# sdmiller/cpu_tsdf

Measured on AMD Instinct MI355X. Metric: integrateCloud throughput, Scene A turntable depth frames, 640x480 -> voxel grid, higher is better.
Workload: dtype f32

## Files before the change

### cpu_tsdf_amd/csrc/tsdf_integrate.hip

```cpp
#include <limits.h>
#include <string.h>
#include <math.h>

#include <algorithm>
#include <cmath>
#include <type_traits>

#include "tsdf_common.h"
#include "tsdf_div.h"
#include "tsdf_buffer.h"
#ifdef TSDF_HIP_TEST_HOOKS
#include "tsdf_hip_test.h"
#endif

#ifndef TSDF_COLOR_PK
#define TSDF_COLOR_PK 2
#endif

typedef float f2 __attribute__((ext_vector_type(2)));
typedef float f4 __attribute__((ext_vector_type(4)));

struct IntegrateArgs {
  float m[12];
  float fxf, fyf, cxf, cyf;
  float hb_u, hb_v;
  float hb_max;
  unsigned kcap, kinc;
  int hinge_fixed;
  int neg_in_window;
  unsigned kmax;
  int wmax_is_int;
  float zmin, zmax;
  float zlo;
  float pos, neg;
  float wmax;
  float pos_over_neg;
  int W, H;
  int ny;
  int plane_rows;
  int qpr;
  int z_global0;
  int zl0;
  int log2TX, TX, TY;
  int rpb;
  unsigned bgra_off;
  int expf_fused_r;
  int ref_cull;
  float cull[24];
  int band_fx, band_fy;
  int implied_d;
  int x_abs0, y_abs0;
  int zfast;
  int64_t pitch;
};

static __device__ __forceinline__ int project_exact(const IntegrateArgs &a, const double *__restrict__ cam,
                                                    float gx, float gy, float gz) {
  const Rcp64 rz = rcp64_prepare((double)gz);
  const int u = (int)(div64((double)gx * cam[0], rz) + cam[2]);
  const int v = (int)(div64((double)gy * cam[1], rz) + cam[3]);
  const bool in = (unsigned)u < (unsigned)a.W && (unsigned)v < (unsigned)a.H;
  return in ? v * a.W + u : -1;
}

template <bool ALLIN = false>
static __device__ __forceinline__ int project_fast(const IntegrateArgs &a, float gx, float gy, float gz,
                                                   bool &ambiguous, uint32_t *margin = nullptr) {
  const float y = __builtin_amdgcn_rcpf(gz);
  const float ru = __builtin_fmaf(gx * a.fxf, y, a.cxf);
  const float rv = __builtin_fmaf(gy * a.fyf, y, a.cyf);
  const int u = (int)ru, v = (int)rv;
  if (ALLIN) {
    *margin = min(__float_as_uint(__builtin_amdgcn_fractf(ru)), __float_as_uint(__builtin_amdgcn_fractf(rv)));
    ambiguous = false;
    return (int)__umul24((unsigned)v, (unsigned)a.W) + u;
  }
  const bool cert = __builtin_amdgcn_fractf(ru) > a.hb_u && __builtin_amdgcn_fractf(rv) > a.hb_v;
  ambiguous = !cert;
  const bool in = (unsigned)u < (unsigned)a.W && (unsigned)v < (unsigned)a.H;
  return in ? (int)__umul24((unsigned)v, (unsigned)a.W) + u : -1;
}

template <int ORDER>
static __device__ __forceinline__ void project_quad_allin(const IntegrateArgs &a, const float (&m)[12], const double *__restrict__ cam,
                                                          const f4 cxv, const f4 ytv, const float (&zt)[3], int (&pix)[4],
                                                          float (&gzs)[4]) {
  const f2 cxa = {cxv.x, cxv.y}, cxb = {cxv.z, cxv.w};
  const float yt[3] = {ytv.x, ytv.y, ytv.z};
  f2 ga[3], gb[3];
#pragma unroll
  for (int q = 0; q < 3; ++q) {
    if (ORDER == TSDF_XFORM_PCL_SSE) {
      ga[q] = cxa * m[4 * q] + yt[q];
      gb[q] = cxb * m[4 * q] + yt[q];
    } else {
      ga[q] = ((cxa * m[4 * q] + yt[q]) + zt[q]) + m[4 * q + 3];
      gb[q] = ((cxb * m[4 * q] + yt[q]) + zt[q]) + m[4 * q + 3];
    }
  }
  const f2 ya = {__builtin_amdgcn_rcpf(ga[2].x), __builtin_amdgcn_rcpf(ga[2].y)};
  const f2 yb = {__builtin_amdgcn_rcpf(gb[2].x), __builtin_amdgcn_rcpf(gb[2].y)};
  const f2 cxf2 = {a.cxf, a.cxf}, cyf2 = {a.cyf, a.cyf};
  const f2 rua = __builtin_elementwise_fma(ga[0] * a.fxf, ya, cxf2), rub = __builtin_elementwise_fma(gb[0] * a.fxf, yb, cxf2);
  const f2 rva = __builtin_elementwise_fma(ga[1] * a.fyf, ya, cyf2), rvb = __builtin_elementwise_fma(gb[1] * a.fyf, yb, cyf2);
  const float ru[4] = {rua.x, rua.y, rub.x, rub.y}, rv[4] = {rva.x, rva.y, rvb.x, rvb.y};
  gzs[0] = ga[2].x, gzs[1] = ga[2].y, gzs[2] = gb[2].x, gzs[3] = gb[2].y;
  uint32_t fu[4], fv[4];
#pragma unroll
  for (int j = 0; j < 4; ++j) {
    fu[j] = __float_as_uint(__builtin_amdgcn_fractf(ru[j]));
    fv[j] = __float_as_uint(__builtin_amdgcn_fractf(rv[j]));
    pix[j] = (int)__umul24((unsigned)(int)rv[j], (unsigned)a.W) + (int)ru[j];
  }
  const uint32_t hb = __float_as_uint(a.hb_max);
  const uint32_t least = min(min(min(fu[0], fv[0]), min(min(fu[1], fv[1]), fu[2])), min(min(fv[2], fu[3]), fv[3]));
  if (!(least > hb)) {
    const float gx[4] = {ga[0].x, ga[0].y, gb[0].x, gb[0].y}, gy[4] = {ga[1].x, ga[1].y, gb[1].x, gb[1].y};
#pragma unroll
    for (int j = 0; j < 4; ++j)
      if (!(min(fu[j], fv[j]) > hb)) pix[j] = project_exact(a, cam, gx[j], gy[j], gzs[j]);
  }
}

static __device__ const uint64_t k_exp2f_tab[32] = {
    0x3ff0000000000000ull, 0x3fefd9b0d3158574ull, 0x3fefb5586cf9890full, 0x3fef9301d0125b51ull, 0x3fef72b83c7d517bull,
    0x3fef54873168b9aaull, 0x3fef387a6e756238ull, 0x3fef1e9df51fdee1ull, 0x3fef06fe0a31b715ull, 0x3feef1a7373aa9cbull,
    0x3feedea64c123422ull, 0x3feece086061892dull, 0x3feebfdad5362a27ull, 0x3feeb42b569d4f82ull, 0x3feeab07dd485429ull,
    0x3feea47eb03a5585ull, 0x3feea09e667f3bcdull, 0x3fee9f75e8ec5f74ull, 0x3feea11473eb0187ull, 0x3feea589994cce13ull,
    0x3feeace5422aa0dbull, 0x3feeb737b0cdc5e5ull, 0x3feec49182a3f090ull, 0x3feed503b23e255dull, 0x3feee89f995ad3adull,
    0x3feeff76f2fb5e47ull, 0x3fef199bdd85529cull, 0x3fef3720dcef9069ull, 0x3fef5818dcfba487ull, 0x3fef7c97337b9b5full,
    0x3fefa4afa2a490daull, 0x3fefd0765b6e4540ull};

static __device__ float tsdf_expf_glibc(float x, bool fused_r) {
  const uint32_t ix = __float_as_uint(x), abstop = (ix >> 20) & 0x7ffu;
  if (abstop >= (0x42b00000u >> 20)) {
    if (ix == 0xff800000u) return 0.f;
    if (abstop >= (0x7f800000u >> 20)) return x + x;
    if (x > 0x1.62e42ep6f) return INFINITY;
    if (x < -0x1.9fe368p6f) return 0.f;
    if (x < -0x1.9d1d9ep6f) return 0x1p-149f;
  }
  const double N = 32., InvLn2N = 0x1.71547652b82fep+0 * N, SHIFT = 0x1.8p+52;
  const double C0 = 0x1.c6af84b912394p-5 / N / N / N, C1 = 0x1.ebfce50fac4f3p-3 / N / N, C2 = 0x1.62e42ff0c52d6p-1 / N;
  const double xd = (double)x;
  double z = InvLn2N * xd;
  double kd = z + SHIFT;
  const uint64_t ki = (uint64_t)__double_as_longlong(kd);
  kd -= SHIFT;
  const double r = fused_r ? __builtin_fma(InvLn2N, xd, -kd) : z - kd;
  const uint64_t t = k_exp2f_tab[ki & 31u] + (ki << 47);
  const double s = __longlong_as_double((long long)t);
  z = C0 * r + C1;
  const double r2 = r * r;
  double y = C2 * r + 1.;
  y = z * r2 + y;
  y = y * s;
  return (float)y;
}

static __device__ __forceinline__ bool reference_cull_keeps(const IntegrateArgs &a, float x, float y, float z) {
  bool keep = true;
#pragma unroll
  for (int k = 0; k < 6; ++k) {
    const float *pl = a.cull + 4 * k;
    keep = keep && ((x * pl[0] + y * pl[1]) + (z * pl[2] + 1.0f * pl[3]) <= 0.f);
  }
  return keep;
}

static __device__ __forceinline__ float div32_fast(float a, const Rcp32 &r) {
  const float q0 = a * r.y;
  const float r0 = __builtin_fmaf(r.nb, q0, a);
  const float q1 = __builtin_fmaf(r0, r.y, q0);
  const float r1 = __builtin_fmaf(r.nb, q1, a);
  return __builtin_fmaf(r1, r.y, q1);
}

static __device__ __forceinline__ bool numerator_ok(float v) {
  const float m = fabsf(v);
  return (m >= 0x1p-100f && m <= 0x1p40f) || __float_as_uint(v) == 0u;
}

template <bool COLOR>
static __device__ __forceinline__ void add_observation_ieee(float &d, float &w, uint32_t &rgb, float dn,
                                                            uint32_t bgra, float wmax) {
  const float wn = 1.f;
  const float wsum = w + wn;
  if (COLOR) {
    uint32_t out = 0;
#pragma unroll
    for (int ch = 0; ch < 3; ++ch) {
      const float c_old = (float)((rgb >> (8 * ch)) & 255u);
      const float c_new = (float)((bgra >> (16 - 8 * ch)) & 255u);
      const float num = w * c_old + wn * c_new;
      out |= ((uint32_t)(uint8_t)(num / wsum)) << (8 * ch);
    }
    rgb = out;
  }
  d = (d * w + dn * wn) / wsum;
  w = wsum;
  if (w > wmax) w = wmax;
}

template <bool COLOR, bool DIST = true>
static __device__ __forceinline__ void add_observation_fast(float &d, float &w, uint32_t &rgb, float dn,
                                                            uint32_t bgra, float wmax, const Rcp32 &rs, uint32_t base = 0u,
                                                            const float *hy_tab = nullptr) {
  const float wsum = w + 1.f;
  if (COLOR) {
#if TSDF_COLOR_PK
    const float hy = hy_tab ? *hy_tab : TSDF_COLOR_PK == 2 ? __builtin_fmaf(0.5f, rs.y, -0.5f) : 0.5f * rs.y;
    const float t0 = __builtin_fmaf(__builtin_fmaf(w, (float)(rgb & 255u), (float)((bgra >> 16) & 255u)), rs.y, hy);
    const float t1 = __builtin_fmaf(__builtin_fmaf(w, (float)((rgb >> 8) & 255u), (float)((bgra >> 8) & 255u)), rs.y, hy);
    const float t2 = __builtin_fmaf(__builtin_fmaf(w, (float)((rgb >> 16) & 255u), (float)(bgra & 255u)), rs.y, hy);
    rgb = __builtin_amdgcn_cvt_pk_u8_f32(t0, 0u, __builtin_amdgcn_cvt_pk_u8_f32(t1, 1u, __builtin_amdgcn_cvt_pk_u8_f32(t2, 2u, base)));
#else
    const float hy = hy_tab ? *hy_tab : 0.5f * rs.y;
    const uint32_t q0 = (uint32_t)__builtin_fmaf(__builtin_fmaf(w, (float)(rgb & 255u), (float)((bgra >> 16) & 255u)), rs.y, hy);
    const uint32_t q1 = (uint32_t)__builtin_fmaf(__builtin_fmaf(w, (float)((rgb >> 8) & 255u), (float)((bgra >> 8) & 255u)), rs.y, hy);
    const uint32_t q2 = (uint32_t)__builtin_fmaf(__builtin_fmaf(w, (float)((rgb >> 16) & 255u), (float)(bgra & 255u)), rs.y, hy);
    rgb = q0 | (q1 << 8) | (q2 << 16) | base;
#endif
  }
  if (DIST) d = div32_fast(d * w + dn, rs);
  w = wsum;
  if (w > wmax) w = wmax;
}

#ifndef TSDF_COLOR_F2
#define TSDF_COLOR_F2 0
#endif
static __device__ __forceinline__ void colour_pair_pk(const f2 w, const uint32_t c0a, const uint32_t c0b, const uint32_t csa, const uint32_t csb,
                                                      const f2 y, const f2 hy, const uint32_t base_a, const uint32_t base_b, uint32_t &cva, uint32_t &cvb) {
  f2 t[3];
#pragma unroll
  for (int ch = 0; ch < 3; ++ch) {
    const f2 o = {(float)((c0a >> (8 * ch)) & 255u), (float)((c0b >> (8 * ch)) & 255u)};
    const f2 n = {(float)((csa >> (16 - 8 * ch)) & 255u), (float)((csb >> (16 - 8 * ch)) & 255u)};
    t[ch] = __builtin_elementwise_fma(__builtin_elementwise_fma(w, o, n), y, hy);
  }
  cva = __builtin_amdgcn_cvt_pk_u8_f32(t[0].x, 0u, __builtin_amdgcn_cvt_pk_u8_f32(t[1].x, 1u, __builtin_amdgcn_cvt_pk_u8_f32(t[2].x, 2u, base_a)));
  cvb = __builtin_amdgcn_cvt_pk_u8_f32(t[0].y, 0u, __builtin_amdgcn_cvt_pk_u8_f32(t[1].y, 1u, __builtin_amdgcn_cvt_pk_u8_f32(t[2].y, 2u, base_b)));
}

static __device__ __forceinline__ bool update_is_safe(float d, float w, float dn) {
  const bool w_ok = fabsf(w - 512.f) <= 512.f && __builtin_amdgcn_fractf(w) == 0.f;
  return w_ok && numerator_ok(d * w + dn);
}


struct BlockCoords {
  unsigned bx, by, bz, gdx, gdy;
};
static __device__ __forceinline__ BlockCoords tsdf_block_coords(int zfast) {
  BlockCoords c;
  c.by = blockIdx.y, c.gdy = gridDim.y;
  c.bx = zfast ? blockIdx.z : blockIdx.x;
  c.bz = zfast ? blockIdx.x : blockIdx.z;
  c.gdx = zfast ? gridDim.z : gridDim.x;
  return c;
}

static __device__ __forceinline__ void tsdf_flags_before(const IntegrateArgs &a, const BlockCoords &bc, const uint8_t *band,
                                                         uint8_t *s_bin, unsigned tid) {
  const int row0 = (int)bc.by * a.rpb * a.TY;
  const int rows = min(a.rpb * a.TY, a.ny - row0);
  const int lf = max(0, a.log2TX - 4), fxb = 1 << lf;
  const int yg0 = (a.y_abs0 + row0) >> 2, yg1 = (a.y_abs0 + row0 + max(rows, 1) - 1) >> 2;
  const int xc0 = (a.x_abs0 + (int)bc.bx * a.TX * 4) >> 6;
  const int n_fl = (yg1 - yg0 + 1) << lf;
  const int n_all = ((a.rpb * a.TY + 3) >> 2) << lf;
  for (int i = (int)tid; i < n_all; i += 256) {
    const int yg = yg0 + (i >> lf), xc = xc0 + (i & (fxb - 1));
    s_bin[i] = i < n_fl && yg < a.band_fy && xc < a.band_fx ? band[((int64_t)(a.zl0 + (int)bc.bz) * a.band_fy + yg) * a.band_fx + xc] : (uint8_t)0;
  }
}
static __device__ __forceinline__ uint64_t tsdf_quiet_passes(const IntegrateArgs &a, const uint8_t *s_bin, unsigned tid) {
  const int lane = (int)(tid & 63u), w0 = (int)(tid & ~63u);
  const int fxb = max(1, a.TX >> 4);
  const int rows_w = max(1, 64 >> a.log2TX), ncell = max(1, min(a.TX, 64) >> 4);
  const int ty0 = w0 >> a.log2TX, c0 = (w0 & (a.TX - 1)) >> 4;
  bool q = lane < a.rpb;
  if (q) {
    for (int rr = 0; rr < rows_w; ++rr)
      for (int c = 0; c < ncell; ++c) q &= s_bin[((ty0 + rr + lane * a.TY) >> 2) * fxb + c0 + c] == 0;
  }
  return __builtin_amdgcn_ballot_w64(q);
}

#ifndef TSDF_GUARD_ON_RESULT
#define TSDF_GUARD_ON_RESULT 1
#endif
#ifndef TSDF_EARLY_VOXEL_LOADS
#define TSDF_EARLY_VOXEL_LOADS 2
#endif

#ifndef TSDF_KTAB
#define TSDF_KTAB 0
#endif
#ifndef TSDF_LEAN_K
#define TSDF_LEAN_K 1
#endif
#ifndef TSDF_SWAR_K
#define TSDF_SWAR_K 1
#endif
#ifndef TSDF_LEAN_BAND
#define TSDF_LEAN_BAND 1
#endif
#ifndef TSDF_AMB_UNROLL
#define TSDF_AMB_UNROLL 1
#endif
#ifndef TSDF_PROJ_F2
#define TSDF_PROJ_F2 1
#endif
struct __attribute__((aligned(16))) KEntry {
  float w;
  float y;
  float hy;
  uint32_t k1;
};
static __device__ __forceinline__ KEntry tsdf_ktab_entry(const IntegrateArgs &a, unsigned k) {
  KEntry e;
  e.w = __builtin_fminf((float)k, a.wmax);
  e.y = rcp32_prepare((float)(k + 1u)).y;
  e.hy = TSDF_COLOR_PK == 2 ? __builtin_fmaf(0.5f, e.y, -0.5f) : 0.5f * e.y;
  e.k1 = min(k << 24, a.kcap) + a.kinc;
  return e;
}
#ifndef TSDF_SKIP_FIXED_HINGE
#define TSDF_SKIP_FIXED_HINGE 1
#endif
#ifndef TSDF_EXP_NO_STORE
#define TSDF_EXP_NO_STORE 0
#endif
#ifndef TSDF_EXP_NO_GATHER
#define TSDF_EXP_NO_GATHER 0
#endif
#ifndef TSDF_EXP_NO_VLOAD
#define TSDF_EXP_NO_VLOAD 0
#endif
#if TSDF_EXP_NO_VLOAD && TSDF_EARLY_VOXEL_LOADS
#error "TSDF_EXP_NO_VLOAD declares the voxel words itself: build it with -DTSDF_EARLY_VOXEL_LOADS=0 (tools/ab_bound.sh does)"
#endif
#if !TSDF_GUARD_ON_RESULT && TSDF_EARLY_VOXEL_LOADS
#error "TSDF_GUARD_ON_RESULT=0 tests the numerator d0 * w0 + dn BEFORE unread distance words are rebuilt from the counts, and with TSDF_EARLY_VOXEL_LOADS those words have no initial value: build that A/B with -DTSDF_EARLY_VOXEL_LOADS=0"
#endif
#ifndef TSDF_GATHER_AUX
#define TSDF_GATHER_AUX 0
#endif
#ifndef TSDF_WPE_MAX
#define TSDF_WPE_MAX 8
#endif
#ifndef TSDF_NO_BAND
#define TSDF_NO_BAND 0
#endif
#ifndef TSDF_BAND_PER_WAVE
#define TSDF_BAND_PER_WAVE 1
#endif
#if TSDF_BAND_PER_WAVE
#define TSDF_BAND_DECL                                                                                     \
  __shared__ __attribute__((aligned(16))) uint8_t s_band_sets[4][1024];                                    \
  reinterpret_cast<u4 *>(&s_band_sets[0][0])[tid] = (u4){0u, 0u, 0u, 0u}
#define TSDF_BAND(i) s_band_sets[threadIdx.x >> 6][i]
#define TSDF_BAND_SYNC() ((void)0)
#define TSDF_BAND_FIRST ((int)(tid & 63u))
#define TSDF_BAND_STEP 64
#else
#define TSDF_BAND_DECL                                                          \
  __shared__ __attribute__((aligned(16))) uint8_t s_band[1024 + 64];            \
  reinterpret_cast<uint32_t *>(s_band)[tid] = 0u, s_band[1024 + (tid & 63u)] = 0
#define TSDF_BAND(i) s_band[i]
#define TSDF_BAND_SYNC() __syncthreads()
#define TSDF_BAND_FIRST ((int)tid)
#define TSDF_BAND_STEP 256
#endif
#ifndef TSDF_RECOMPUTE_PX
#define TSDF_RECOMPUTE_PX 1
#endif
#ifndef TSDF_WPE_PACKED
#define TSDF_WPE_PACKED 7
#endif
#ifndef TSDF_WPE_PACKED_COLOR
#define TSDF_WPE_PACKED_COLOR 8
#endif
#define TSDF_WPE_OF(ORDER, COLOR, FASTPROJ, COUNT, PACKED, ALLIN) \
  ((ALLIN) && !(COUNT) && (PACKED) && (COLOR) && (FASTPROJ) ? TSDF_WPE_PACKED_COLOR : (ALLIN) && !(COUNT) && ((PACKED) || !(COLOR)) ? TSDF_WPE_PACKED : TSDF_WPE_GENERAL)
#ifndef TSDF_WPE_GENERAL
#define TSDF_WPE_GENERAL 7
#endif
#ifndef TSDF_PHASE_TIMER
#define TSDF_PHASE_TIMER 0
#endif
#if TSDF_PHASE_TIMER
#define TSDF_NPHASE 16
__device__ unsigned long long g_phase[1024 * TSDF_NPHASE];
static __device__ __forceinline__ uint32_t tsdf_clock_lo() {
  uint64_t t;
  asm volatile("s_memtime %0\n\ts_waitcnt lgkmcnt(0)" : "=s"(t)::"memory");
  return (uint32_t)t;
}
#define TSDF_NACC 9
#define PT_DECL                                                   \
  uint32_t pt_acc[TSDF_NACC];                                     \
  _Pragma("unroll") for (int i_ = 0; i_ < TSDF_NACC; ++i_) asm volatile("v_mov_b32 %0, 0" : "=v"(pt_acc[i_])); \
  const unsigned pt_blk = (blockIdx.x + blockIdx.y * gridDim.x + blockIdx.z * gridDim.x * gridDim.y) & 1023u; \
  uint32_t pt_prev = tsdf_clock_lo();                             \
  const uint32_t pt_t0 = pt_prev
#define PT_MARK(k)                           \
  do {                                       \
    const uint32_t pt_now = tsdf_clock_lo(); \
    pt_acc[k] += pt_now - pt_prev;           \
    pt_prev = pt_now;                        \
  } while (0)
                    \

#define PT_MARK_OUT(k)                                                                                 \
  do {                                                                                                 \
    const uint32_t pt_now = tsdf_clock_lo();                                                           \
    if ((threadIdx.x & 63u) == 0u) atomicAdd(&g_phase[pt_blk * TSDF_NPHASE + (k)], (unsigned long long)(pt_now - pt_prev)); \
    pt_prev = pt_now;                                                                                  \
  } while (0)
#define PT_COUNT(k) pt_acc[k] += 1u
#define PT_DEP4(a_, b_, c_, d_) asm volatile("" ::"v"(a_), "v"(b_), "v"(c_), "v"(d_) : "memory")
#define PT_DEP1(a_) asm volatile("" ::"v"(a_) : "memory")
#define PT_FLUSH()                                                                                       \
  do {                                                                                                   \
    const uint32_t pt_now = tsdf_clock_lo();                                                             \
    if ((threadIdx.x & 63u) == 0u) {                                                                     \
      atomicAdd(&g_phase[pt_blk * TSDF_NPHASE + 15], (unsigned long long)(pt_now - pt_t0));              \
      _Pragma("unroll") for (int i_ = 0; i_ < TSDF_NACC; ++i_)                                           \
          atomicAdd(&g_phase[pt_blk * TSDF_NPHASE + i_], (unsigned long long)pt_acc[i_]);                \
    }                                                                                                    \
  } while (0)
#else
#define PT_DECL
#define PT_MARK(k)
#define PT_MARK_OUT(k)
#define PT_COUNT(k)
#define PT_DEP4(a_, b_, c_, d_)
#define PT_DEP1(a_)
#define PT_FLUSH()
#endif
template <int ORDER, bool COLOR, bool FASTPROJ, bool COUNT, bool PACKED, bool ALLIN = false, bool LIVE = false>
static __global__ void __launch_bounds__(256) __attribute__((amdgpu_waves_per_eu(TSDF_WPE_OF(ORDER, COLOR, FASTPROJ, COUNT, PACKED, ALLIN) < TSDF_WPE_MAX ? TSDF_WPE_OF(ORDER, COLOR, FASTPROJ, COUNT, PACKED, ALLIN) : TSDF_WPE_MAX, TSDF_WPE_MAX)))
k_integrate(const IntegrateArgs a, float *__restrict__ D, float *__restrict__ Wt, uint32_t *__restrict__ RGB,
            uint8_t *__restrict__ K8, const float *__restrict__ depth, const double *__restrict__ cam,
            const float *__restrict__ ctrx, const float *__restrict__ ctry, const float *__restrict__ ctrz,
            unsigned long long *__restrict__ n_obs, const uint8_t *__restrict__ live, uint8_t *__restrict__ band,
            const uint32_t *__restrict__ row_iv) {
  static_assert(!(ALLIN && LIVE), "the ALLIN instance knows no row intervals");
  const BlockCoords bc = tsdf_block_coords(a.zfast);
  PT_DECL;
  bool strad = false;
  if (LIVE) {
    const unsigned flag = live[bc.bx + bc.gdx * (bc.by + bc.gdy * bc.bz)];
    if (flag == 0u) return;
    strad = flag == 2u;
  }
  const unsigned tid = threadIdx.x;
#if TSDF_KTAB
  __shared__ KEntry s_tab[PACKED ? 256 : 1];
#else
  __shared__ f2 s_rcp[256];
#endif
  __shared__ f4 s_yt[256];
  constexpr bool F2 = TSDF_PROJ_F2 && ALLIN && FASTPROJ;
  constexpr bool LEAN_K1 = TSDF_LEAN_K && !TSDF_KTAB && TSDF_COLOR_PK == 2 && PACKED && COLOR;
  __shared__ f4 s_cx[F2 ? 256 : 1];
  __shared__ uint32_t s_iv[LIVE ? 256 : 1];
  TSDF_BAND_DECL;
#if TSDF_KTAB
  if (PACKED) s_tab[tid] = tsdf_ktab_entry(a, tid);
#else
  if (PACKED) {
    const KEntry e = tsdf_ktab_entry(a, tid);
    s_rcp[tid] = (f2){e.y, e.hy};
  }
#endif
  {
    const int yy = (int)bc.by * a.rpb * a.TY + (int)tid;
    {
      const float cy_ = ctry[yy < a.ny ? yy : a.ny - 1], cz_ = ctrz[a.z_global0 + (int)bc.bz];
      f4 t = {0.f, 0.f, 0.f, 0.f};
#pragma unroll
      for (int q = 0; q < 3; ++q)
        t[q] = ORDER == TSDF_XFORM_PCL_SSE ? cy_ * a.m[4 * q + 1] + (cz_ * a.m[4 * q + 2] + a.m[4 * q + 3]) : a.m[4 * q + 1] * cy_;
      s_yt[tid] = t;
    }
    if (F2) {
      const int xq_ = (int)bc.bx * a.TX + (int)(tid & (unsigned)(a.TX - 1));
      if (xq_ < a.qpr) s_cx[tid] = *reinterpret_cast<const f4 *>(ctrx + xq_ * 4);
    }
    if (LIVE && strad) s_iv[tid] = yy < a.ny ? row_iv[(int64_t)bc.bz * a.ny + yy] : 0u;
  }
  __shared__ uint8_t s_bin[PACKED ? 1024 : 1];
  if (PACKED && a.implied_d) tsdf_flags_before(a, bc, band, s_bin, tid);
  __syncthreads();
  const uint64_t quiet = PACKED && a.implied_d ? tsdf_quiet_passes(a, s_bin, tid) : 0ull;
  PT_MARK_OUT(9);
  const int tx = (int)(tid & (unsigned)(a.TX - 1));
  const int ty = (int)(tid >> a.log2TX);
  const int xq = (int)bc.bx * a.TX + tx;
  const int zl = (int)bc.bz;
  const Rcp32 rneg = rcp32_prepare(a.neg);
  unsigned cnt = 0, chg = 0, imp = 0, rdb = 0;
  const int row0 = (int)bc.by * a.rpb * a.TY;
  const int rows = min(a.rpb * a.TY, a.ny - row0);
  const int64_t e0 = ((int64_t)(a.zl0 + zl) * a.plane_rows + row0) * a.pitch;
  const unsigned span = (unsigned)rows * (unsigned)a.pitch;
  const rsrc_t rsD = make_rsrc(D + e0, span * 4u);
  const rsrc_t rsW = make_rsrc(PACKED ? D : Wt + e0, PACKED ? 0u : span * 4u);
  const rsrc_t rsC = make_rsrc(COLOR ? RGB + e0 : (uint32_t *)D, COLOR ? span * 4u : 0u);
  const rsrc_t rsK = make_rsrc(PACKED && !COLOR ? K8 + e0 : (uint8_t *)D, PACKED && !COLOR ? span : 0u);
  const unsigned npix = (unsigned)a.W * (unsigned)a.H;
  const rsrc_t rsF = make_rsrc(depth, COLOR ? a.bgra_off + npix * 4u : npix * 4u);
  const i4_rsrc rsFi = make_rsrc_2d(depth, 4u, 0xffffffffu);
  if (xq < a.qpr) {
    const int x4 = xq * 4;
    const float cz = ctrz[a.z_global0 + zl];
    const float4 cx4 = *reinterpret_cast<const float4 *>(ctrx + x4);
    const float cxs[4] = {cx4.x, cx4.y, cx4.z, cx4.w};
    float px_[4][3], zt[3];
#pragma unroll
    for (int r = 0; r < 3; ++r) {
#pragma unroll
      for (int j = 0; j < 4; ++j) px_[j][r] = cxs[j] * a.m[4 * r];
      zt[r] = ORDER == TSDF_XFORM_PCL_SSE ? cz * a.m[4 * r + 2] + a.m[4 * r + 3] : a.m[4 * r + 2] * cz;
    }
    const unsigned voff = (unsigned)(ty * (int)a.pitch + x4) * 4u;
    const unsigned row_step = (unsigned)a.TY * (unsigned)a.pitch * 4u;
#if TSDF_EARLY_VOXEL_LOADS
    bool pred_obs = true;
#endif
    for (int r = 0; r < a.rpb; ++r) {
      const int y = row0 + ty + r * a.TY;
      if (y >= a.ny) break;
      unsigned iv_lo = 0u, iv_len = 0u;
      if (LIVE && strad) {
        const uint32_t iv = s_iv[ty + r * a.TY];
        iv_lo = iv & 0xffffu, iv_len = iv >> 16;
        if (!((unsigned)(x4 + 3) - iv_lo < iv_len + 3u)) continue;
      }
      const unsigned soff = (unsigned)r * row_step;
      const f4 ytv = s_yt[ty + r * a.TY];
      const float yt[3] = {ytv.x, ytv.y, ytv.z};
#if TSDF_RECOMPUTE_PX
      float px[4][3];
      if constexpr (!F2) {
        float cxr[4] = {cxs[0], cxs[1], cxs[2], cxs[3]};
#pragma unroll
        for (int j = 0; j < 4; ++j) asm volatile("" : "+v"(cxr[j]));
#pragma unroll
        for (int q = 0; q < 3; ++q)
#pragma unroll
          for (int j = 0; j < 4; ++j) px[j][q] = cxr[j] * a.m[4 * q];
      }
#else
      const float (&px)[4][3] = px_;
#endif
      auto transform = [&](int j, int q) -> float {
        if (ORDER == TSDF_XFORM_PCL_SSE) return px[j][q] + yt[q];
        return ((px[j][q] + yt[q]) + zt[q]) + a.m[4 * q + 3];
      };
      int pix[4];
      float gzs[4];
      bool any = false, lowz = false;
      if constexpr (F2) {
        asm volatile("" ::: "memory");
        project_quad_allin<ORDER>(a, a.m, cam, s_cx[tid], ytv, zt, pix, gzs);
        PT_DEP4(pix[0], pix[1], pix[2], pix[3]);
        PT_MARK(0);
      } else {
      unsigned amb_mask = 0;
      uint32_t margin[4] = {0u, 0u, 0u, 0u};
#pragma unroll
      for (int j = 0; j < 4; ++j) {
        const float gx = transform(j, 0), gy = transform(j, 1), gz = transform(j, 2);
        const bool in = ALLIN || (gz > a.zlo && !(gz > a.zmax) && (!LIVE || !strad || (unsigned)(x4 + j) - iv_lo < iv_len));
        gzs[j] = gz;
        if (!ALLIN) lowz |= in && gz < 0x1p-14f;
        int p;
        if (FASTPROJ) {
          bool amb;
          p = project_fast<ALLIN>(a, gx, gy, gz, amb, &margin[j]);
          if (amb && in) amb_mask |= 1u << j;
        } else {
          p = project_exact(a, cam, gx, gy, in ? gz : 1.f);
        }
        pix[j] = in ? p : -1;
        any |= in;
      }
      if (!ALLIN && !any) continue;
      if (ALLIN && FASTPROJ) {
        const uint32_t hb = __float_as_uint(a.hb_max);
        if (!(min(min(margin[0], margin[1]), min(margin[2], margin[3])) > hb)) {
#pragma unroll
          for (int j = 0; j < 4; ++j)
            if (!(margin[j] > hb)) amb_mask |= 1u << j;
        }
      }
#if TSDF_AMB_UNROLL
      if (FASTPROJ && amb_mask) {
#pragma unroll
        for (int j = 0; j < 4; ++j)
          if (amb_mask >> j & 1u) pix[j] = project_exact(a, cam, transform(j, 0), transform(j, 1), transform(j, 2));
      }
#else
      while (FASTPROJ && amb_mask) {
        const int j = __builtin_ctz(amb_mask);
        amb_mask &= amb_mask - 1;
        float g[3];
#pragma unroll
        for (int q = 0; q < 3; ++q)
          g[q] = j == 0 ? transform(0, q) : j == 1 ? transform(1, q) : j == 2 ? transform(2, q) : transform(3, q);
        const int p = project_exact(a, cam, g[0], g[1], g[2]);
        if (j == 0) pix[0] = p;
        if (j == 1) pix[1] = p;
        if (j == 2) pix[2] = p;
        if (j == 3) pix[3] = p;
      }
#endif
      }
#if TSDF_EARLY_VOXEL_LOADS
      constexpr bool EARLY = PACKED;
      const bool d_read = !PACKED || !(r < 64 && (quiet >> r & 1ull));
      u4 d4;
      asm volatile("" : "=v"(d4));
      u4 w4 = {0u, 0u, 0u, 0u}, c4 = {0u, 0u, 0u, 0u};
      uint32_t k4 = 0u;
      const bool ask_early = EARLY && (TSDF_EARLY_VOXEL_LOADS != 2 || pred_obs);
      if (ask_early) {
        if (d_read) d4 = bload128(rsD, voff, soff);
        if (COLOR) c4 = bload128(rsC, voff, soff);
        if (!COLOR) k4 = bload32(rsK, voff >> 2, soff >> 2);
        if (COUNT) rdb += (d_read ? 16u : 0u) + (COLOR ? 16u : 4u);
      }
#endif
      float zs[4];
      uint32_t cs[4] = {0u, 0u, 0u, 0u};
#pragma unroll
      for (int j = 0; j < 4; ++j) {
        if (TSDF_EXP_NO_GATHER) {
          zs[j] = 1e3f + (float)(pix[j] & 1);
          cs[j] = 0x00406080u + (unsigned)pix[j];
        } else if (ALLIN) {
          zs[j] = __uint_as_float(tsdf_struct_buffer_load_u32(rsFi, pix[j], 0, 0, TSDF_GATHER_AUX));
          if (COLOR) cs[j] = tsdf_struct_buffer_load_u32(rsFi, pix[j], 0, (int)a.bgra_off, TSDF_GATHER_AUX);
        } else {
          zs[j] = __uint_as_float(bload32(rsF, (unsigned)pix[j] << 2, 0u));
          if (COLOR) cs[j] = bload32(rsF, (unsigned)pix[j] << 2, a.bgra_off);
        }
      }
// ... 96 lines not shown
          kw[j] = COLOR ? c0[j] : (k4 << (24 - 8 * j));
#if TSDF_KTAB
          const KEntry e = s_tab[kw[j] >> 24];
          w0[j] = e.w, ky[j] = e.y, khy[j] = e.hy, k1[j] = e.k1;
#else
          if (TSDF_LEAN_K && ALLIN) {
            w0[j] = (float)(kw[j] >> 24);
            if (COLOR) asm volatile("" : "+v"(w0[j]));
          } else {
            w0[j] = __builtin_fminf((float)(kw[j] >> 24), a.wmax);
          }
          k1[j] = LEAN_K1 ? min(kw[j], a.kcap | 0xffffffu) + a.kinc : min(kw[j] & 0xff000000u, a.kcap) + a.kinc;
#endif
        }
      }
      bool safe = true;
      if (!PACKED) {
#pragma unroll
        for (int j = 0; j < 4; ++j) safe &= !act[j] || update_is_safe(d0[j], w0[j], dn[j]);
      }
#if !TSDF_GUARD_ON_RESULT
      else {
#pragma unroll
        for (int j = 0; j < 4; ++j)
          safe &= !act[j] || ((a.wmax_is_int || kw[j] < (a.kmax << 24)) && numerator_ok(d0[j] * w0[j] + dn[j]));
      }
#endif
      bool d_moves = true;
#if TSDF_SKIP_FIXED_HINGE
      if (PACKED && a.hinge_fixed) {
        bool off_hinge = any_div;
        if (d_read) {
#pragma unroll
          for (int j = 0; j < 4; ++j) off_hinge |= (ALLIN || act[j]) && d0u[j] != __float_as_uint(a.pos_over_neg);
        } else {
#pragma unroll
          for (int j = 0; j < 4; ++j) off_hinge |= (ALLIN || act[j]) && kw[j] < 0x01000000u;
          if (TSDF_SWAR_K && ALLIN && !COLOR) off_hinge = any_div || ((k4 - 0x01010101u) & ~k4 & 0x80808080u) != 0u;
        }
        d_moves = __builtin_amdgcn_ballot_w64(off_hinge) != 0ull;
      }
#endif
      if (PACKED && !d_read && d_moves) {
#pragma unroll
        for (int j = 0; j < 4; ++j) {
          d0u[j] = kw[j] < 0x01000000u ? 0xbf800000u : __float_as_uint(a.pos_over_neg);
          d0[j] = __uint_as_float(d0u[j]);
        }
      }
      bool d_touched = false;
      if (safe) {
        Rcp32 rs[4];
#pragma unroll
        for (int j = 0; j < 4; ++j) dv[j] = d0[j], wv[j] = w0[j], cv[j] = c0[j];
        constexpr bool QUAD_COLOR = TSDF_COLOR_F2 && COLOR && PACKED && TSDF_COLOR_PK == 2 && !TSDF_KTAB;
        if constexpr (QUAD_COLOR) {
#pragma unroll
          for (int j = 0; j < 4; j += 2) {
            const f2 yh0 = s_rcp[kw[j] >> 24], yh1 = s_rcp[kw[j + 1] >> 24];
            rs[j].nb = -(w0[j] + 1.f), rs[j + 1].nb = -(w0[j + 1] + 1.f);
            rs[j].y = yh0.x, rs[j + 1].y = yh1.x;
            colour_pair_pk((f2){w0[j], w0[j + 1]}, c0[j], c0[j + 1], cs[j], cs[j + 1], (f2){yh0.x, yh1.x}, (f2){yh0.y, yh1.y}, k1[j], k1[j + 1],
                           cv[j], cv[j + 1]);
          }
        } else
        if (COLOR || !PACKED || d_moves)
#pragma unroll
        for (int j = 0; j < 4; ++j) {
          if (PACKED) {
            rs[j].nb = -(w0[j] + 1.f);
#if TSDF_KTAB
            rs[j].y = ky[j];
#else
            const f2 yh = s_rcp[kw[j] >> 24];
            rs[j].y = yh.x, khy[j] = yh.y;
#endif
          } else {
            rs[j] = rcp32_prepare(w0[j] + 1.f);
          }
          add_observation_fast<COLOR, false>(dv[j], wv[j], cv[j], dn[j], cs[j], a.wmax, rs[j], COLOR ? k1[j] : 0u, PACKED ? &khy[j] : nullptr);
        }
        if (d_moves) {
          d_touched = true;
          if (!TSDF_NO_BAND && any_div) TSDF_BAND(((ty + r * a.TY) >> 2) * max(1, a.TX >> 4) + (tx >> 4)) = 1;
#pragma unroll
          for (int j = 0; j < 4; ++j) dv[j] = div32_fast(d0[j] * w0[j] + dn[j], rs[j]);
#if TSDF_GUARD_ON_RESULT
          if (PACKED) {
#pragma unroll
            for (int j = 0; j < 4; ++j)
              safe &= !act[j] || ((ALLIN || a.wmax_is_int || kw[j] < (a.kmax << 24)) && __builtin_amdgcn_classf(dv[j], 0x108));
          }
#endif
        }
      }
      if (!safe) {
        d_touched = true;
        if (!TSDF_NO_BAND && any_div) TSDF_BAND(((ty + r * a.TY) >> 2) * max(1, a.TX >> 4) + (tx >> 4)) = 1;
        asm volatile("");
#pragma unroll
        for (int j = 0; j < 4; ++j) {
          dv[j] = d0[j];
          wv[j] = w0[j];
          cv[j] = c0[j] & 0xffffffu;
          add_observation_ieee<COLOR>(dv[j], wv[j], cv[j], dn[j], cs[j], a.wmax);
          if (COLOR) cv[j] |= k1[j] & 0xff000000u;
        }
      }
      PT_DEP4(dv[0], dv[1], cv[0], cv[1]);
      PT_MARK(6);
      uint32_t diff_w = 0u, diff_c = 0u, k4n = 0u;
      uint32_t wn_u[4];
      const uint32_t c_before[4] = {c0[0], c0[1], c0[2], c0[3]};
      if (d_touched) {
        uint32_t diff_d = 0u, dn_u[4];
#pragma unroll
        for (int j = 0; j < 4; ++j) {
          dn_u[j] = act[j] ? __float_as_uint(dv[j]) : d0u[j];
          diff_d |= dn_u[j] ^ d0u[j];
          if (COUNT) chg += dn_u[j] != d0u[j] ? 4u : 0u;
        }
        if (diff_d && !TSDF_EXP_NO_STORE) bstore128(rsD, voff, soff, (u4){dn_u[0], dn_u[1], dn_u[2], dn_u[3]});
      }
#pragma unroll
      for (int j = 0; j < 4; ++j) {
        if (PACKED && !COLOR && !TSDF_SWAR_K) k4n |= (act[j] ? k1[j] : (kw[j] & 0xff000000u)) >> (24 - 8 * j);
        wn_u[j] = act[j] ? __float_as_uint(wv[j]) : w0u[j];
        cv[j] = act[j] ? cv[j] : c0[j];
        diff_w |= wn_u[j] ^ w0u[j];
        diff_c |= cv[j] ^ c0[j];
        cnt += act[j] ? 1u : 0u;
        if (COUNT && PACKED) imp += act[j] && !d_read ? 1u : 0u;
        if (COUNT)
          chg += (!PACKED && wn_u[j] != w0u[j] ? 4u : 0u) + (COLOR && cv[j] != c_before[j] ? 4u : 0u);
      }
      if (PACKED && !COLOR && TSDF_SWAR_K) {
        const uint32_t km2 = a.kmax * 0x00010001u;
        const uint32_t te = ((k4 & 0x00ff00ffu) | 0x01000100u) - km2, to = (((k4 >> 8) & 0x00ff00ffu) | 0x01000100u) - km2;
        const uint32_t lt = ((~te >> 8) & 0x00010001u) | (((~to >> 8) & 0x00010001u) << 8);
        const uint32_t actb = (act[0] ? 0x00000001u : 0u) | (act[1] ? 0x00000100u : 0u) | (act[2] ? 0x00010000u : 0u) | (act[3] ? 0x01000000u : 0u);
        k4n = k4 + (lt & actb);
      }
      if (COUNT && PACKED && !COLOR) chg += (unsigned)__popc(((k4n ^ k4) | ((k4n ^ k4) >> 1) | ((k4n ^ k4) >> 2) | ((k4n ^ k4) >> 3) |
                                                            ((k4n ^ k4) >> 4) | ((k4n ^ k4) >> 5) | ((k4n ^ k4) >> 6) | ((k4n ^ k4) >> 7)) & 0x01010101u);
      if (!PACKED && diff_w) bstore128(rsW, voff, soff, (u4){wn_u[0], wn_u[1], wn_u[2], wn_u[3]});
      if (TSDF_EXP_NO_STORE) {
        if ((cv[0] ^ cv[1] ^ cv[2] ^ cv[3]) == 0x12345678u) bstore32(rsD, voff, soff, cv[0] ^ diff_w);
      } else
      if (COLOR && diff_c) bstore128(rsC, voff, soff, (u4){cv[0], cv[1], cv[2], cv[3]});
      if (PACKED && !COLOR && k4n != k4) bstore32(rsK, voff >> 2, soff >> 2, k4n);
      PT_MARK(7);
    }
  }
  PT_MARK_OUT(10);
  if (!TSDF_NO_BAND && band) {
    TSDF_BAND_SYNC();
    const int lf = max(0, a.log2TX - 4), fxb = 1 << lf;
    const int yg0 = (a.y_abs0 + row0) >> 2, yg1 = (a.y_abs0 + row0 + max(rows, 1) - 1) >> 2;
    const int xc0 = (a.x_abs0 + (int)bc.bx * a.TX * 4) >> 6;
    const int n_fl = (yg1 - yg0 + 1) << lf;
    for (int i = TSDF_BAND_FIRST; i < n_fl; i += TSDF_BAND_STEP) {
      const int yg = yg0 + (i >> lf), xc = xc0 + (i & (fxb - 1));
      if (TSDF_BAND(i) && yg < a.band_fy && xc < a.band_fx) band[((int64_t)(a.zl0 + zl) * a.band_fy + yg) * a.band_fx + xc] = 1;
    }
  }
  PT_MARK_OUT(12);
  PT_FLUSH();
  if (COUNT) {
    __shared__ unsigned s_cnt, s_chg, s_imp, s_rdb;
    if (tid == 0) s_cnt = s_chg = s_imp = s_rdb = 0;
    __syncthreads();
    if (cnt) atomicAdd(&s_cnt, cnt);
    if (chg) atomicAdd(&s_chg, chg);
    if (imp) atomicAdd(&s_imp, imp);
    if (rdb) atomicAdd(&s_rdb, rdb);
    __syncthreads();
    if (tid == 0 && (s_cnt || s_rdb)) {
      const unsigned b = bc.bx + bc.by * bc.gdx + bc.bz * bc.gdx * bc.gdy;
      if (s_cnt) atomicAdd(n_obs + (b & 1023u), (unsigned long long)s_cnt);
      if (s_chg) atomicAdd(n_obs + 1024u + (b & 1023u), (unsigned long long)s_chg);
      if (s_imp) atomicAdd(n_obs + 2048u + (b & 1023u), (unsigned long long)s_imp);
// ... 884 lines not shown
  const int ya = by * c.by_rows, yb = min(c.ny, ya + c.by_rows) - 1;
  bool any = box_may_be_observed(c, ctrx[xa], ctrx[xb], ctry[ya], ctry[yb], ctrz[c.z_global0 + bz]), all = true;
  if (any) {
    any = false;
    for (int y = ya; y <= yb; ++y) {
      const uint32_t iv = row_iv[(int64_t)bz * c.ny + y];
      const int lo = (int)(iv & 0xffffu), len = (int)(iv >> 16);
      any |= len > 0 && lo <= xb && lo + len - 1 >= xa;
      all &= lo <= xa && lo + len - 1 >= xb;
    }
  }
  live[b] = !any ? 0 : all ? 1 : 2;
}

static float f32_ulp(float v) {
  const float a = fabsf(v);
  return nextafterf(a, INFINITY) - a;
}

struct IntegrateHost {
  IntegrateArgs a;
  float band_u, band_v;
  double fx, fy;
  int planes;
};

static IntegrateHost make_args(tsdf_handle h, const float T[12]) {
  const tsdf_params &p = h->p;
  IntegrateHost hh;
  IntegrateArgs &a = hh.a;
  for (int i = 0; i < 12; ++i) a.m[i] = T[i];
  hh.fx = p.fx;
  hh.fy = p.fy;
  a.fxf = (float)p.fx;
  a.fyf = (float)p.fy;
  {
    auto band = [](double c, int n) {
      const double q = std::max(fabs(c) + 1.0, fabs((double)n + 1.0 - c));
      const double e = q * (2.0 / 16777216.0 + 1.0 / 4194304.0) * 1.0000005 + ((double)n + 2.0) / 16777216.0 +
                       2.0 * f32_ulp((float)c) + 1e-9;
      return nextafterf((float)(1.5 * e), INFINITY);
    };
    hh.band_u = band(p.cx, p.image_width);
    hh.band_v = band(p.cy, p.image_height);
    a.cxf = (float)(p.cx + (double)hh.band_u);
    a.cyf = (float)(p.cy + (double)hh.band_v);
    a.hb_u = nextafterf(2.f * hh.band_u, INFINITY);
    a.hb_v = nextafterf(2.f * hh.band_v, INFINITY);
    a.hb_max = std::max(a.hb_u, a.hb_v);
  }
  a.zmin = p.min_sensor_dist;
  a.zlo = p.min_sensor_dist > 0.f ? nextafterf(p.min_sensor_dist, -INFINITY) : 0.f;
  a.zmax = p.max_sensor_dist;
  a.pos = p.max_dist_pos;
  a.neg = p.max_dist_neg;
  a.wmax = p.max_weight;
  a.kmax = h->kmax;
  a.kcap = h->kmax ? (h->kmax - 1u) << 24 : 0u;
  a.kinc = h->kmax ? 0x01000000u : 0u;
  a.wmax_is_int = p.max_weight == floorf(p.max_weight);
  a.pos_over_neg = p.max_dist_pos / p.max_dist_neg;
  {
    const volatile float pv = a.pos_over_neg;
    bool fixed = h->packed && a.wmax_is_int && std::isnormal(a.pos_over_neg);
    for (unsigned k = 0; fixed && k <= h->kmax; ++k) {
      const volatile float w = fminf((float)k, p.max_weight);
      const volatile float num = pv * w;
      const volatile float sum = num + pv;
      const volatile float den = w + 1.f;
      const volatile float q = sum / den;
      fixed = q == pv;
    }
    a.hinge_fixed = fixed ? 1 : 0;
  }
  a.neg_in_window = p.max_dist_neg >= 0x1p-20f && p.max_dist_neg <= 0x1p20f && p.max_dist_pos <= 0x1p20f;
  a.W = p.image_width;
  a.H = p.image_height;
  a.ny = h->ny;
  a.plane_rows = h->ny;
  a.qpr = (h->nx + 3) / 4;
  hh.planes = h->z_end - h->z_begin;
  a.z_global0 = h->z_begin;
  a.zl0 = h->z_begin - h->z_first;
  int l2 = 0;
  while ((1 << l2) < a.qpr && l2 < 8) ++l2;
  a.log2TX = l2;
  a.TX = 1 << l2;
  a.TY = 256 / a.TX;
  a.rpb = std::max(1, std::min(tsdf_tuning().rows_per_block, 256) / a.TY);
  a.rpb = std::max(1, std::min(a.rpb, (a.ny + a.TY - 1) / a.TY));
  a.pitch = h->pitch;
  a.expf_fused_r = h->expf_fused_r;
  a.ref_cull = h->ref_cull ? 1 : 0;
  for (int i = 0; i < 24; ++i) a.cull[i] = h->ref_cull ? h->cull_planes[i] : 0.f;
  a.band_fx = h->band_fx;
  a.band_fy = h->band_fy;
  a.x_abs0 = a.y_abs0 = 0;
  a.zfast = 0;
  return hh;
}

struct PlainObs {
  int pix;
  float z;
  float dn;
  int64_t vi;
};

template <int ORDER>
static __device__ __forceinline__ bool plain_observe(const IntegrateArgs &a, const double *__restrict__ cam,
                                                     const float *__restrict__ ctrx, const float *__restrict__ ctry,
                                                     const float *__restrict__ ctrz, const float *__restrict__ depth, PlainObs *o) {
  const int x = (int)(blockIdx.x * 256u + threadIdx.x);
  const int y = (int)blockIdx.y, zl = (int)blockIdx.z;
  if (!(x < (int)a.pitch)) return false;
  const float cx = ctrx[x], cy = ctry[y], cz = ctrz[a.z_global0 + zl];
  float g[3];
#pragma unroll
  for (int q = 0; q < 3; ++q)
    g[q] = ORDER == TSDF_XFORM_PCL_SSE ? cx * a.m[4 * q] + (cy * a.m[4 * q + 1] + (cz * a.m[4 * q + 2] + a.m[4 * q + 3]))
                                       : ((a.m[4 * q] * cx + a.m[4 * q + 1] * cy) + a.m[4 * q + 2] * cz) + a.m[4 * q + 3];
  const bool in = !(g[2] < a.zmin || g[2] > a.zmax) && g[2] > 0.f &&
                  (!a.ref_cull || reference_cull_keeps(a, cx, cy, cz));
  o->pix = in ? project_exact(a, cam, g[0], g[1], g[2]) : -1;
  if (o->pix < 0) return false;
  o->z = depth[o->pix];
  const float dn = o->z - g[2];
  if (isnan(o->z) || dn < -a.neg) return false;
  o->dn = dn > a.pos ? a.pos_over_neg : dn / a.neg;
  o->vi = ((int64_t)(a.zl0 + zl) * a.plane_rows + y) * a.pitch + x;
  return true;
}

static __device__ __forceinline__ void plain_count(bool observed, unsigned long long *__restrict__ n_obs) {
  if (!n_obs) return;
  const unsigned long long m = __ballot(observed);
  if ((threadIdx.x & 63u) == 0u && m)
    atomicAdd(n_obs + ((blockIdx.x + blockIdx.y * gridDim.x + blockIdx.z * gridDim.x * gridDim.y) & 1023u),
              (unsigned long long)__popcll(m));
}

template <int ORDER>
static __global__ void __launch_bounds__(256)
k_integrate_rgbn(const IntegrateArgs a, float *__restrict__ D, float *__restrict__ Wt, uint32_t *__restrict__ RGB,
                 float *__restrict__ RN, float *__restrict__ GN, float *__restrict__ BN, float *__restrict__ IN,
                 const float *__restrict__ depth, const uint32_t *__restrict__ bgra, const double *__restrict__ cam,
                 const float *__restrict__ ctrx, const float *__restrict__ ctry, const float *__restrict__ ctrz,
                 unsigned long long *__restrict__ n_obs) {
  PlainObs o;
  const bool observed = plain_observe<ORDER>(a, cam, ctrx, ctry, ctrz, depth, &o);
  if (observed) {
    const int64_t vi = o.vi;
    const uint32_t c = bgra[o.pix];
    const float r = (float)((c >> 16) & 255u), gch = (float)((c >> 8) & 255u), b = (float)(c & 255u);
    float w = Wt[vi], d = D[vi];
    const float wn = 1.f;
    const float wsum = w + wn;
    const float i = sqrtf(r * r + gch * gch + b * b);
    const float rf = r / i, gf = gch / i, bf = b / i;
    const float rn = (w * RN[vi] + wn * rf) / wsum;
    const float gn = (w * GN[vi] + wn * gf) / wsum;
    const float bn = (w * BN[vi] + wn * bf) / wsum;
    const float im = (w * IN[vi] + wn * i) / wsum;
    RN[vi] = rn;
    GN[vi] = gn;
    BN[vi] = bn;
    IN[vi] = im;
    RGB[vi] = ((uint32_t)(int)(rn * im) & 255u) | (((uint32_t)(int)(gn * im) & 255u) << 8) |
              (((uint32_t)(int)(bn * im) & 255u) << 16);
    uint32_t unused = 0;
    add_observation_ieee<false>(d, w, unused, o.dn, 0u, a.wmax);
    D[vi] = d;
// ... 1512 lines not shown
```

Before: 667,300.

## Precompute x-column transform products in LDS and shrink per-block row arrays

The x-column products cx*m[4q] for all three rows are now computed once per block into shared memory (s_px) and reloaded each row, so the per-row multiply is gone. The per-row LDS arrays (s_yt, s_iv, band sets, s_bin) are capped at 64 rows, and rows_per_block is clamped to match. The row loop is rewritten around a byte offset with a wave-uniform trip count and a helper for band marking, and the minimum tile width is raised to 4. This trades three times more LDS for the x products and a smaller row batch per block for less arithmetic and a smaller LDS footprint, which may raise occupancy. Fewer rows per block could add launch and setup overhead.

```diff
diff --git a/cpu_tsdf_amd/csrc/tsdf_integrate.hip b/cpu_tsdf_amd/csrc/tsdf_integrate.hip
--- a/cpu_tsdf_amd/csrc/tsdf_integrate.hip
+++ b/cpu_tsdf_amd/csrc/tsdf_integrate.hip
@@ -82,20 +82,31 @@
 }
 
 template <int ORDER>
+static __device__ __forceinline__ void project_quad_products(const IntegrateArgs &a, const float (&m)[12], const double *__restrict__ cam,
+                                                             const f2 (&pa)[3], const f2 (&pb)[3], const f4 ytv, const float (&zt)[3],
+                                                             int (&pix)[4], float (&gzs)[4]);
+template <int ORDER>
 static __device__ __forceinline__ void project_quad_allin(const IntegrateArgs &a, const float (&m)[12], const double *__restrict__ cam,
                                                           const f4 cxv, const f4 ytv, const float (&zt)[3], int (&pix)[4],
                                                           float (&gzs)[4]) {
   const f2 cxa = {cxv.x, cxv.y}, cxb = {cxv.z, cxv.w};
+  const f2 pa[3] = {cxa * m[0], cxa * m[4], cxa * m[8]}, pb[3] = {cxb * m[0], cxb * m[4], cxb * m[8]};
+  project_quad_products<ORDER>(a, m, cam, pa, pb, ytv, zt, pix, gzs);
+}
+template <int ORDER>
+static __device__ __forceinline__ void project_quad_products(const IntegrateArgs &a, const float (&m)[12], const double *__restrict__ cam,
+                                                             const f2 (&pa)[3], const f2 (&pb)[3], const f4 ytv, const float (&zt)[3],
+                                                             int (&pix)[4], float (&gzs)[4]) {
   const float yt[3] = {ytv.x, ytv.y, ytv.z};
   f2 ga[3], gb[3];
 #pragma unroll
   for (int q = 0; q < 3; ++q) {
     if (ORDER == TSDF_XFORM_PCL_SSE) {
-      ga[q] = cxa * m[4 * q] + yt[q];
-      gb[q] = cxb * m[4 * q] + yt[q];
+      ga[q] = pa[q] + yt[q];
+      gb[q] = pb[q] + yt[q];
     } else {
-      ga[q] = ((cxa * m[4 * q] + yt[q]) + zt[q]) + m[4 * q + 3];
-      gb[q] = ((cxb * m[4 * q] + yt[q]) + zt[q]) + m[4 * q + 3];
+      ga[q] = ((pa[q] + yt[q]) + zt[q]) + m[4 * q + 3];
+      gb[q] = ((pb[q] + yt[q]) + zt[q]) + m[4 * q + 3];
     }
   }
   const f2 ya = {__builtin_amdgcn_rcpf(ga[2].x), __builtin_amdgcn_rcpf(ga[2].y)};
@@ -261,6 +272,8 @@
   return c;
 }
 
+constexpr int TSDF_BLOCK_ROWS_MAX = 64;
+constexpr int TSDF_BLOCK_CELLS_MAX = (TSDF_BLOCK_ROWS_MAX / 4) * 16;
 static __device__ __forceinline__ void tsdf_flags_before(const IntegrateArgs &a, const BlockCoords &bc, const uint8_t *band,
                                                          uint8_t *s_bin, unsigned tid) {
   const int row0 = (int)bc.by * a.rpb * a.TY;
@@ -359,9 +372,11 @@
 #endif
 #if TSDF_BAND_PER_WAVE
 #define TSDF_BAND_DECL                                                                                     \
-  __shared__ __attribute__((aligned(16))) uint8_t s_band_sets[4][1024];                                    \
-  reinterpret_cast<u4 *>(&s_band_sets[0][0])[tid] = (u4){0u, 0u, 0u, 0u}
+  static_assert(4 * TSDF_BLOCK_CELLS_MAX == 256 * 4, "one word per thread clears the four sets");          \
+  __shared__ __attribute__((aligned(16))) uint8_t s_band_sets[4][TSDF_BLOCK_CELLS_MAX];                    \
+  reinterpret_cast<uint32_t *>(&s_band_sets[0][0])[tid] = 0u
 #define TSDF_BAND(i) s_band_sets[threadIdx.x >> 6][i]
+#define TSDF_BAND_OF(t, i) s_band_sets[0][((t) >> 6) * (unsigned)TSDF_BLOCK_CELLS_MAX + (i)]
 #define TSDF_BAND_SYNC() ((void)0)
 #define TSDF_BAND_FIRST ((int)(tid & 63u))
 #define TSDF_BAND_STEP 64
@@ -370,12 +385,10 @@
   __shared__ __attribute__((aligned(16))) uint8_t s_band[1024 + 64];            \
   reinterpret_cast<uint32_t *>(s_band)[tid] = 0u, s_band[1024 + (tid & 63u)] = 0
 #define TSDF_BAND(i) s_band[i]
+#define TSDF_BAND_OF(t, i) s_band[i]
 #define TSDF_BAND_SYNC() __syncthreads()
 #define TSDF_BAND_FIRST ((int)tid)
 #define TSDF_BAND_STEP 256
-#endif
-#ifndef TSDF_RECOMPUTE_PX
-#define TSDF_RECOMPUTE_PX 1
 #endif
 #ifndef TSDF_WPE_PACKED
 #define TSDF_WPE_PACKED 7
@@ -463,11 +476,11 @@
 #else
   __shared__ f2 s_rcp[256];
 #endif
-  __shared__ f4 s_yt[256];
+  __shared__ f4 s_yt[TSDF_BLOCK_ROWS_MAX];
   constexpr bool F2 = TSDF_PROJ_F2 && ALLIN && FASTPROJ;
   constexpr bool LEAN_K1 = TSDF_LEAN_K && !TSDF_KTAB && TSDF_COLOR_PK == 2 && PACKED && COLOR;
-  __shared__ f4 s_cx[F2 ? 256 : 1];
-  __shared__ uint32_t s_iv[LIVE ? 256 : 1];
+  __shared__ f4 s_px[F2 ? 3 : 1][F2 ? 256 : 1];
+  __shared__ uint32_t s_iv[LIVE ? TSDF_BLOCK_ROWS_MAX : 1];
   TSDF_BAND_DECL;
 #if TSDF_KTAB
   if (PACKED) s_tab[tid] = tsdf_ktab_entry(a, tid);
@@ -479,21 +492,25 @@
 #endif
   {
     const int yy = (int)bc.by * a.rpb * a.TY + (int)tid;
-    {
+    if (tid < (unsigned)TSDF_BLOCK_ROWS_MAX) {
       const float cy_ = ctry[yy < a.ny ? yy : a.ny - 1], cz_ = ctrz[a.z_global0 + (int)bc.bz];
       f4 t = {0.f, 0.f, 0.f, 0.f};
 #pragma unroll
       for (int q = 0; q < 3; ++q)
         t[q] = ORDER == TSDF_XFORM_PCL_SSE ? cy_ * a.m[4 * q + 1] + (cz_ * a.m[4 * q + 2] + a.m[4 * q + 3]) : a.m[4 * q + 1] * cy_;
       s_yt[tid] = t;
+      if (LIVE && strad) s_iv[tid] = yy < a.ny ? row_iv[(int64_t)bc.bz * a.ny + yy] : 0u;
     }
     if (F2) {
       const int xq_ = (int)bc.bx * a.TX + (int)(tid & (unsigned)(a.TX - 1));
-      if (xq_ < a.qpr) s_cx[tid] = *reinterpret_cast<const f4 *>(ctrx + xq_ * 4);
-    }
-    if (LIVE && strad) s_iv[tid] = yy < a.ny ? row_iv[(int64_t)bc.bz * a.ny + yy] : 0u;
-  }
-  __shared__ uint8_t s_bin[PACKED ? 1024 : 1];
+      if (xq_ < a.qpr) {
+        const f4 cx_ = *reinterpret_cast<const f4 *>(ctrx + xq_ * 4);
+#pragma unroll
+        for (int q = 0; q < 3; ++q) s_px[q][tid] = cx_ * a.m[4 * q];
+      }
+    }
+  }
+  __shared__ uint8_t s_bin[PACKED ? TSDF_BLOCK_CELLS_MAX : 1];
   if (PACKED && a.implied_d) tsdf_flags_before(a, bc, band, s_bin, tid);
   __syncthreads();
   const uint64_t quiet = PACKED && a.implied_d ? tsdf_quiet_passes(a, s_bin, tid) : 0ull;
@@ -515,38 +532,48 @@
   const unsigned npix = (unsigned)a.W * (unsigned)a.H;
   const rsrc_t rsF = make_rsrc(depth, COLOR ? a.bgra_off + npix * 4u : npix * 4u);
   const i4_rsrc rsFi = make_rsrc_2d(depth, 4u, 0xffffffffu);
+  const int ty_w = (int)((tid & ~63u) >> a.log2TX);
+  const int n_rows = __builtin_amdgcn_readfirstlane(max(0, (rows - ty_w + a.TY - 1) >> (8 - a.log2TX)));
+  const bool rows_differ = a.log2TX < 6;
   if (xq < a.qpr) {
     const int x4 = xq * 4;
     const float cz = ctrz[a.z_global0 + zl];
     const float4 cx4 = *reinterpret_cast<const float4 *>(ctrx + x4);
     const float cxs[4] = {cx4.x, cx4.y, cx4.z, cx4.w};
-    float px_[4][3], zt[3];
-#pragma unroll
-    for (int r = 0; r < 3; ++r) {
-#pragma unroll
-      for (int j = 0; j < 4; ++j) px_[j][r] = cxs[j] * a.m[4 * r];
-      zt[r] = ORDER == TSDF_XFORM_PCL_SSE ? cz * a.m[4 * r + 2] + a.m[4 * r + 3] : a.m[4 * r + 2] * cz;
-    }
+    float zt[3];
+#pragma unroll
+    for (int r = 0; r < 3; ++r) zt[r] = ORDER == TSDF_XFORM_PCL_SSE ? cz * a.m[4 * r + 2] + a.m[4 * r + 3] : a.m[4 * r + 2] * cz;
     const unsigned voff = (unsigned)(ty * (int)a.pitch + x4) * 4u;
     const unsigned row_step = (unsigned)a.TY * (unsigned)a.pitch * 4u;
 #if TSDF_EARLY_VOXEL_LOADS
     bool pred_obs = true;
 #endif
-    for (int r = 0; r < a.rpb; ++r) {
-      const int y = row0 + ty + r * a.TY;
-      if (y >= a.ny) break;
+    unsigned yb = (unsigned)ty * 16u;
+    auto mark_band = [&](const unsigned yb_) {
+      unsigned t_ = tid;
+      asm volatile("" : "+v"(t_));
+      TSDF_BAND_OF(t_, (yb_ >> 6) * (unsigned)max(1, a.TX >> 4) + ((t_ & (unsigned)(a.TX - 1)) >> 4)) = 1;
+    };
+    const unsigned yb_step = (unsigned)a.TY * 16u, yb_end = (unsigned)rows * 16u;
+    for (int r = 0; r < n_rows; ++r, yb += yb_step) {
+      asm volatile("" : "+v"(yb));
+      if (rows_differ && yb >= yb_end) continue;
       unsigned iv_lo = 0u, iv_len = 0u;
       if (LIVE && strad) {
-        const uint32_t iv = s_iv[ty + r * a.TY];
+        const uint32_t iv = s_iv[yb >> 4];
         iv_lo = iv & 0xffffu, iv_len = iv >> 16;
         if (!((unsigned)(x4 + 3) - iv_lo < iv_len + 3u)) continue;
       }
       const unsigned soff = (unsigned)r * row_step;
-      const f4 ytv = s_yt[ty + r * a.TY];
+      const f4 ytv = *reinterpret_cast<const f4 *>(reinterpret_cast<const char *>(s_yt) + yb);
       const float yt[3] = {ytv.x, ytv.y, ytv.z};
-#if TSDF_RECOMPUTE_PX
       float px[4][3];
-      if constexpr (!F2) {
+      f4 pxv[3];
+      if constexpr (F2) {
+        asm volatile("" ::: "memory");
+#pragma unroll
+        for (int q = 0; q < 3; ++q) pxv[q] = s_px[q][tid];
+      } else {
         float cxr[4] = {cxs[0], cxs[1], cxs[2], cxs[3]};
 #pragma unroll
         for (int j = 0; j < 4; ++j) asm volatile("" : "+v"(cxr[j]));
@@ -555,9 +582,6 @@
 #pragma unroll
           for (int j = 0; j < 4; ++j) px[j][q] = cxr[j] * a.m[4 * q];
       }
-#else
-      const float (&px)[4][3] = px_;
-#endif
       auto transform = [&](int j, int q) -> float {
         if (ORDER == TSDF_XFORM_PCL_SSE) return px[j][q] + yt[q];
         return ((px[j][q] + yt[q]) + zt[q]) + a.m[4 * q + 3];
@@ -566,8 +590,9 @@
       float gzs[4];
       bool any = false, lowz = false;
       if constexpr (F2) {
-        asm volatile("" ::: "memory");
-        project_quad_allin<ORDER>(a, a.m, cam, s_cx[tid], ytv, zt, pix, gzs);
+        const f2 pa[3] = {{pxv[0].x, pxv[0].y}, {pxv[1].x, pxv[1].y}, {pxv[2].x, pxv[2].y}};
+        const f2 pb[3] = {{pxv[0].z, pxv[0].w}, {pxv[1].z, pxv[1].w}, {pxv[2].z, pxv[2].w}};
+        project_quad_products<ORDER>(a, a.m, cam, pa, pb, ytv, zt, pix, gzs);
         PT_DEP4(pix[0], pix[1], pix[2], pix[3]);
         PT_MARK(0);
       } else {
@@ -830,7 +855,7 @@
         }
         if (d_moves) {
           d_touched = true;
-          if (!TSDF_NO_BAND && any_div) TSDF_BAND(((ty + r * a.TY) >> 2) * max(1, a.TX >> 4) + (tx >> 4)) = 1;
+          if (!TSDF_NO_BAND && any_div) mark_band(yb);
 #pragma unroll
           for (int j = 0; j < 4; ++j) dv[j] = div32_fast(d0[j] * w0[j] + dn[j], rs[j]);
 #if TSDF_GUARD_ON_RESULT
@@ -844,7 +869,7 @@
       }
       if (!safe) {
         d_touched = true;
-        if (!TSDF_NO_BAND && any_div) TSDF_BAND(((ty + r * a.TY) >> 2) * max(1, a.TX >> 4) + (tx >> 4)) = 1;
+        if (!TSDF_NO_BAND && any_div) mark_band(yb);
         asm volatile("");
 #pragma unroll
         for (int j = 0; j < 4; ++j) {
@@ -1895,12 +1920,13 @@
   hh.planes = h->z_end - h->z_begin;
   a.z_global0 = h->z_begin;
   a.zl0 = h->z_begin - h->z_first;
-  int l2 = 0;
+  int l2 = 2;
   while ((1 << l2) < a.qpr && l2 < 8) ++l2;
   a.log2TX = l2;
   a.TX = 1 << l2;
   a.TY = 256 / a.TX;
-  a.rpb = std::max(1, std::min(tsdf_tuning().rows_per_block, 256) / a.TY);
+  static_assert(256 / 4 <= TSDF_BLOCK_ROWS_MAX, "one pass of the narrowest tile fits the per-row LDS arrays");
+  a.rpb = std::max(1, std::min(tsdf_tuning().rows_per_block, TSDF_BLOCK_ROWS_MAX) / a.TY);
   a.rpb = std::max(1, std::min(a.rpb, (a.ny + a.TY - 1) / a.TY));
   a.pitch = h->pitch;
   a.expf_fused_r = h->expf_fused_r;
```

After: 663,700. No clear change (-0.6%).
